# charlesknipp/sequential_monte_carlo

Measured on AMD Instinct MI355X. Metric: particle-steps/sec, higher is better.
Workload: dtype f64; 1 GPU; LinearGaussian1D bootstrap filter Nx=2^20 T=1000 (BASELINE configs[1]); n_theta_per_gpu=1, n_x=1048576, T=1000, seg=2048, resident_kernel=False, resampler=multinomial

## Files before the change

sequential_monte_carlo_amd/csrc/smc_kernels.h:

```cpp
#pragma once
#include "smc_spec.h"
#include <cstddef>
#include <type_traits>

namespace smc {

constexpr int WAVE = 64;
__host__ __device__ constexpr int lds_pad(int i) { return i + ((i >> 5) << 1); }
__host__ __device__ constexpr int lds_probe_off(int s) { return s >= 32 ? lds_pad(s - 32) + 31 : s - 1; }
__host__ __device__ constexpr int lds_step_inc(int s) { return s >= 32 ? lds_pad(s) : s; }
__host__ __device__ constexpr int lds_unpad(int pp) { return pp - 2 * (pp / 34); }
__host__ __device__ constexpr int lds_padded_len(int n) { return n + (n >> 4) + 8; }

typedef __attribute__((address_space(3))) const char lds_byte;
typedef __attribute__((address_space(3))) const uint64_t lds_u64;
typedef __attribute__((address_space(3))) const double lds_f64;
__device__ __forceinline__ lds_byte* lds_ptr(const void* p) { return (lds_byte*)p; }
__device__ __forceinline__ uint64_t lds_load_u64(lds_byte* p) { return *(lds_u64*)p; }

typedef unsigned long long nt_v2u64 __attribute__((ext_vector_type(2)));
template <class T>
__device__ __forceinline__ void store_out(T* p, const T& val) {
    static_assert(sizeof(T) == 16, "16-byte stores");
    __builtin_nontemporal_store(*reinterpret_cast<const nt_v2u64*>(&val), reinterpret_cast<nt_v2u64*>(p));
// ... 34 lines not shown
    int want_s2;
    const unsigned char* skip;
    const int32_t* order;
    const int32_t* n_active;
    int sum_np, sum_comp, sum_mom, sum_unw;
    uint64_t sum_p64[8];
    double* sum_q;
    double* sum_m;
    int abl;
    int prop_kind;
    unsigned long long* dbg;
    PropRow* prop;
};

#ifdef SMC_ABLATE
#define SMC_ABL(v, bit) (((v).abl >> (bit)) & 1)
#define SMC_STAMP(v, k)                                                                                   \
    do {                                                                                                  \
        if ((v).dbg && threadIdx.x == 0)                                                                  \
            (v).dbg[((size_t)blockIdx.y * gridDim.x + blockIdx.x) * 8 + (k)] = __builtin_amdgcn_s_memrealtime(); \
    } while (0)
#define SMC_CLOCK() __builtin_amdgcn_s_memrealtime()
#define SMC_STAMP_AT(v, k, clk)                                                                           \
    do {                                                                                                  \
        if ((v).dbg && threadIdx.x == 0)                                                                  \
            (v).dbg[((size_t)blockIdx.y * gridDim.x + blockIdx.x) * 8 + (k)] = (clk);                     \
    } while (0)
#define SMC_STAMP_START(v, t_draw, t_entry)                                                               \
    do {                                                                                                  \
        if ((v).dbg && threadIdx.x == 0) {                                                                \
            unsigned long long* d_ = (v).dbg + ((size_t)gridDim.y * gridDim.x + (size_t)blockIdx.y * gridDim.x + blockIdx.x) * 8; \
            d_[0] = (t_draw); d_[1] = (t_entry);                                                          \
        }                                                                                                 \
    } while (0)
#define SMC_ORDER_AFTER(x) asm volatile("" : : "v"(x))
#else
#define SMC_ORDER_AFTER(x) do { } while (0)
#define SMC_ABL(v, bit) 0
#define SMC_STAMP(v, k) do { } while (0)
#define SMC_STAMP_AT(v, k, clk) do { (void)(clk); } while (0)
#define SMC_CLOCK() 0ull
#define SMC_STAMP_START(v, t_draw, t_entry) do { (void)(t_draw); (void)(t_entry); } while (0)
#endif
__device__ __forceinline__ void host_emit(const FilterView& v, int th, double z, double logmu, double ess) {
    if (!v.host_out) return;
    v.host_out[th] = z;
    v.host_out[(size_t)v.ntheta + th] = logmu;
    v.host_out[2 * (size_t)v.ntheta + th] = ess;
    if (v.host_seq) {
        __threadfence_system();
        __hip_atomic_store(&v.host_out[3 * (size_t)v.ntheta + th], (double)v.host_seq, __ATOMIC_RELEASE, __HIP_MEMORY_SCOPE_SYSTEM);
    }
}
constexpr int QMAX = 8;
__host__ __device__ inline uint64_t order_key(double x) {
    const uint64_t b = d2bits(x);
    return (b >> 63) ? ~b : (b | 0x8000000000000000ULL);
}
__host__ __device__ inline double key_value(uint64_t k) { return bits2d((k >> 63) ? (k & 0x7fffffffffffffffULL) : ~k); }
__host__ __device__ inline uint64_t prob_to_u64(double p) {
    if (!(p > 0.0)) return 0;
    if (p >= 1.0) return ~(uint64_t)0;
    return (uint64_t)(p * TWO_P64);
}
struct Q7Rank { int64_t j; double g; };
__host__ __device__ inline Q7Rank q7_rank(int64_t n, double p) {
    const double h = (double)n * p + (1.0 - p);
    int64_t j = (int64_t)h;
    j = j > n - 1 ? n - 1 : (j < 1 ? 1 : j);
    double g = h - (double)j;
    g = g > 1.0 ? 1.0 : (g < 0.0 ? 0.0 : g);
    Q7Rank r; r.j = j; r.g = g;
    return r;
}
__host__ __device__ inline double q7_interp(double a, double b, double g) {
    const bool fin = (a - a == 0.0) && (b - b == 0.0);
    return fin ? a + g * (b - a) : (1.0 - g) * a + g * b;
}
__host__ __device__ inline double q7_level(double p) { return p > 0.0 ? (p < 1.0 ? p : 1.0) : 0.0; }


#define SMC_PRIO(ph) __builtin_amdgcn_s_setprio((short)(3 - (ph)))

template <int CTRL, int ROW_MASK>
__device__ __forceinline__ uint32_t dpp_u32(uint32_t old, uint32_t v) {
    return (uint32_t)__builtin_amdgcn_update_dpp((int)old, (int)v, CTRL, ROW_MASK, 0xf, false);
}
template <int CTRL>
__device__ __forceinline__ uint64_t dpp_add_u64(uint64_t v) {
    uint32_t lo = (uint32_t)v, hi = (uint32_t)(v >> 32);
#define SMC_DPP_ADD64(MOD)                                                                                  \
    asm volatile("s_nop 1\n\tv_add_co_u32_dpp %0, vcc, %0, %0 " MOD "\n\ts_nop 1\n\tv_addc_co_u32_dpp %1, vcc, %1, %1, vcc " MOD \
                 : "+v"(lo), "+v"(hi) : : "vcc")
    static_assert(CTRL == 0x111 || CTRL == 0x112 || CTRL == 0x114 || CTRL == 0x118 || CTRL == 0x142 || CTRL == 0x143, "DPP control");
    if (CTRL == 0x111) SMC_DPP_ADD64("row_shr:1 row_mask:0xf bank_mask:0xf bound_ctrl:1");
    if (CTRL == 0x112) SMC_DPP_ADD64("row_shr:2 row_mask:0xf bank_mask:0xf bound_ctrl:1");
    if (CTRL == 0x114) SMC_DPP_ADD64("row_shr:4 row_mask:0xf bank_mask:0xf bound_ctrl:1");
    if (CTRL == 0x118) SMC_DPP_ADD64("row_shr:8 row_mask:0xf bank_mask:0xf bound_ctrl:1");
    if (CTRL == 0x142) SMC_DPP_ADD64("row_bcast:15 row_mask:0xa bank_mask:0xf");
    if (CTRL == 0x143) SMC_DPP_ADD64("row_bcast:31 row_mask:0xc bank_mask:0xf");
#undef SMC_DPP_ADD64
    return ((uint64_t)hi << 32) | lo;
}
__device__ __forceinline__ uint64_t wave_incl_scan(uint64_t v, int ) {
    v = dpp_add_u64<0x111>(v);
    v = dpp_add_u64<0x112>(v);
    v = dpp_add_u64<0x114>(v);
    v = dpp_add_u64<0x118>(v);
    v = dpp_add_u64<0x142>(v);
    v = dpp_add_u64<0x143>(v);
    return v;
}
__device__ __forceinline__ uint32_t wave_incl_scan_u32(uint32_t v) {
    v += dpp_u32<0x111, 0xf>(0u, v);
    v += dpp_u32<0x112, 0xf>(0u, v);
    v += dpp_u32<0x114, 0xf>(0u, v);
    v += dpp_u32<0x118, 0xf>(0u, v);
    v += dpp_u32<0x142, 0xa>(0u, v);
    v += dpp_u32<0x143, 0xc>(0u, v);
    return v;
}
__device__ __forceinline__ uint64_t wave_incl_scan_52(uint64_t v) {
    const uint32_t lo = wave_incl_scan_u32((uint32_t)v & 0x3ffffffu);
    const uint32_t hi = wave_incl_scan_u32((uint32_t)(v >> 26));
    return ((uint64_t)hi << 26) + lo;
}
__device__ __forceinline__ uint64_t readlane_u64(uint64_t v, int l) {
    const uint32_t lo = (uint32_t)__builtin_amdgcn_readlane((int)(uint32_t)v, l);
    const uint32_t hi = (uint32_t)__builtin_amdgcn_readlane((int)(uint32_t)(v >> 32), l);
    return ((uint64_t)hi << 32) | lo;
}
__device__ __forceinline__ uint64_t wave_sum(uint64_t v) { return readlane_u64(wave_incl_scan(v, 0), WAVE - 1); }
template <int NW>
__device__ __forceinline__ void wave_totals(const uint64_t* tot, int lane, int wave, uint64_t& off, uint64_t& all) {
    static_assert(NW >= 1 && NW <= 16 && (NW & (NW - 1)) == 0, "wave count");
    uint64_t t = tot[lane & (NW - 1)];
    if (NW > 1) t = dpp_add_u64<0x111>(t);
    if (NW > 2) t = dpp_add_u64<0x112>(t);
    if (NW > 4) t = dpp_add_u64<0x114>(t);
    if (NW > 8) t = dpp_add_u64<0x118>(t);
    const int ws = __builtin_amdgcn_readfirstlane(wave);
    all = readlane_u64(t, NW - 1);
    const uint64_t prev = readlane_u64(t, ws > 0 ? ws - 1 : 0);
    off = ws > 0 ? prev : 0;
}

struct U128 {
    uint64_t lo, hi;
};
__device__ __forceinline__ U128 add128(U128 a, U128 b) {
    U128 r;
    r.lo = a.lo + b.lo;
    r.hi = a.hi + b.hi + (r.lo < a.lo ? 1u : 0u);
    return r;
}
__device__ __forceinline__ U128 sq128(uint64_t q) {
    U128 r;
    r.hi = __umul64hi(q, q);
    r.lo = q * q;
    return r;
}
template <int CTRL>
__device__ __forceinline__ U128 dpp_add_u128(U128 v) {
    uint32_t w0 = (uint32_t)v.lo, w1 = (uint32_t)(v.lo >> 32), w2 = (uint32_t)v.hi, w3 = (uint32_t)(v.hi >> 32);
#define SMC_DPP_ADD128(MOD)                                                                                       \
    asm volatile("s_nop 1\n\tv_add_co_u32_dpp %0, vcc, %0, %0 " MOD "\n\ts_nop 1\n\tv_addc_co_u32_dpp %1, vcc, %1, %1, vcc " MOD \
// ... 555 lines not shown
    double y;
    if constexpr (BYV) { prm = *prm0; y = yval; }
    else { prm = v.params[th]; y = v.y ? v.y[t] : yval; }
    PropRow prw;
    if constexpr (GUIDED) prw = v.prop[th];
    const uint32_t n32 = ea.n32;
    double xr[D] = {};
    if constexpr (COND) {
        uint32_t lane0 = 0u;
        if constexpr (D == 1) asm volatile("" : "+v"(lane0));
#pragma unroll
        for (int c = 0; c < D; ++c) xr[c] = xrow[(size_t)c * v.ntheta + th + lane0];
    }
    const uint64_t* Cprev = ea.C + (size_t)th * ((size_t)nseg * SEG);
    const double* xprev = v.x[cur];
    uint64_t* scr;
    SMC_PRIO(0);

    uint64_t F0 = 0, F1 = 0;
    if (MULTI && !SYS) {
        const uint64_t* Fb = ea.brow + (size_t)th * ((size_t)nseg + 1) + sb;
        F0 = Fb[0];
        F1 = Fb[1];
    }
    const TablePre tpre = (MULTI && !GTAB) ? table_preload<THREADS, RPT>(v, (const double*)ea.rec0, (const uint64_t*)ea.rec1, nseg, cur, th, emit_prev == 1 && sb == 0)
                                           : TablePre{-inf(), 0, 0, 0, -inf(), 0};
    unsigned long long t_draw = 0;
#pragma unroll
    for (int k = 0; k < NP; ++k) {
        if (SYS) { rr[2 * k] = rr[2 * k + 1] = 0; continue; }
        const uint32_t pg = (uint32_t)((seg0 >> 1) + tid + k * THREADS);
        rw[k] = draw(seed, pg, stream, t, SLOT_RESAMPLE);
        if (k == 0) {
            SMC_ORDER_AFTER(rw[0].v[3]);
            t_draw = SMC_CLOCK();
        }
        if (SMC_ABL(v, 3)) rw[k] = u32x4{{pg * 2654435761u, pg ^ t, pg * 40503u, ~pg}};
        rr[2 * k] = ((uint64_t)rw[k].v[1] << 32) | rw[k].v[0];
        rr[2 * k + 1] = ((uint64_t)rw[k].v[3] << 32) | rw[k].v[2];
    }
#ifdef SMC_ABLATE
    if (SMC_ABL(v, 8) && (blockIdx.x & 8)) {
        __builtin_amdgcn_s_sleep(127);
        __builtin_amdgcn_s_sleep(127);
    }
#endif
    const uint32_t m_blk = (seg0 + SEG < n32 ? seg0 + SEG : n32) - seg0;
    const bool ragged = seg0 + SEG > n32;
    uint32_t kk[NQ];
#pragma unroll
    for (int i = 0; i < NQ; ++i) kk[i] = 2 * (tid + (i >> 1) * THREADS) + (i & 1);
    if (ragged) {
        asm volatile("; ragged");
#pragma unroll
        for (int i = 0; i < NQ; ++i) kk[i] = (seg0 + kk[i] < n32 ? seg0 + kk[i] : n32 - 1) - seg0;
    }
    uint64_t Tg[NQ];

    constexpr bool SPEC = MULTI && NSTAGE == 3;
    ulonglong2 stg[NSTAGE][NP];
    int spec_lo = 0;
    if (SPEC) {
        spec_lo = sb - 1 < 0 ? 0 : sb - 1;
        spec_lo = spec_lo + NSTAGE > nseg ? (nseg - NSTAGE < 0 ? 0 : nseg - NSTAGE) : spec_lo;
#pragma unroll
        for (int sg = 0; sg < NSTAGE; ++sg) {
#pragma unroll
            for (int k = 0; k < NP; ++k) stg[sg][k] = ulonglong2{0, 0};
            if (spec_lo + sg < nseg) {
                const ulonglong2* src = reinterpret_cast<const ulonglong2*>(Cprev + (size_t)(spec_lo + sg) * SEG);
#pragma unroll
                for (int k = 0; k < NP; ++k) stg[sg][k] = src[tid + k * THREADS];
            }
        }
    }

    ulonglong2 stg1[NP];
    constexpr bool EARLY1 = D == 1;
#pragma unroll
    for (int k = 0; k < NP; ++k)
        stg1[k] = (!MULTI && EARLY1) ? reinterpret_cast<const ulonglong2*>(Cprev)[tid + k * THREADS] : ulonglong2{0, 0};

    constexpr bool LATE_Z = D >= 3 && NP >= 2 && !SYS;
    double z[NP][NZ][2];
#pragma unroll
    for (int k = 0; k < NP; ++k) {
        if (LATE_Z) break;
        const uint32_t pg = (uint32_t)((seg0 >> 1) + tid + k * THREADS);
#pragma unroll
        for (int c = 0; c < NZ; ++c) {
            if (SMC_ABL(v, 2)) { z[k][c][0] = 1e-3 * (double)(pg & 1023); z[k][c][1] = -z[k][c][0]; }
            else if (SMC_ABL(v, 6)) { const u32x4 w4 = draw(seed, pg, stream, t, SLOT_NORMAL0 + c); z[k][c][0] = 1e-9 * (double)w4.v[0]; z[k][c][1] = 1e-9 * (double)w4.v[2]; }
            else box_muller(draw(seed, pg, stream, t, SLOT_NORMAL0 + c), z[k][c][0], z[k][c][1]);
            if (SYS) asm volatile("" : "+v"(z[k][c][0]), "+v"(z[k][c][1]));
        }
    }


    uint64_t alive;
    uint64_t Sseg[NQ];
    int bseg[NQ];
    uint64_t* Cst = nullptr;
    int blo = 0;
    const int tab_p2 = GTAB ? 0 : v.nseg_p2;
    if (MULTI) {
        TableLds L = carve(smem, tab_p2);
        if (GTAB) {
            const size_t p2 = (size_t)1 << (32 - __builtin_clz((unsigned)(nseg - 1)));
            L.Dcum = (uint64_t*)ea.rec0 + (size_t)th * p2;
            L.sh = (int*)ea.rec1 + (size_t)th * p2;
        }
        scr = L.scr;
        uint64_t* sysw = L.scr + scr_words(THREADS, NP) - 8;
        if (SYS && tid == 0) {
            const u32x4 uw = draw(seed, 0u, stream, t, SLOT_SYS);
            sysw[0] = ((uint64_t)uw.v[1] << 32) | uw.v[0];
        }
        const bool emitter = emit_prev && sb == 0;
        const bool emit_totals = emitter && emit_prev == 2;
        const int s_hi = spec_lo + NSTAGE - 1 < v.nseg - 1 ? spec_lo + NSTAGE - 1 : v.nseg - 1;
        const bool use_fast = SPEC && (GTAB || ((!emitter || emit_totals) && v.nseg_p2 <= RPT * THREADS));
        uint64_t P0 = 0, Dc[NSTAGE];
        int shw[NSTAGE];
        if (GTAB) {
            alive = L.Dcum[v.nseg - 1];
            if (SPEC) {
                P0 = spec_lo ? L.Dcum[spec_lo - 1] : 0;
#pragma unroll
                for (int i = 0; i < NSTAGE; ++i) { Dc[i] = L.Dcum[spec_lo + i]; shw[i] = L.sh[spec_lo + i]; }
            }
            if (SYS) __syncthreads();
        } else if (use_fast) {
            double Kw;
            alive = window_prologue<THREADS, NSTAGE, RPT>(v, L.scr, tpre, spec_lo, P0, Dc, shw, Kw);
            if (emit_totals && tid == 0) emit_from_totals(v, th, Kw, alive, t == 1u, t - 1u);
        } else {
            alive = table_prologue<THREADS>(v, cur, th, L, emitter, t == 1u, t - 1u, RPT == 1 ? &tpre : nullptr);
        }
        SMC_STAMP(v, 1);
        SMC_PRIO(1);
        SysBase sbase{};
        uint64_t Tfirst, Tlast, lo_ = 0;
        if (SYS) {
            sbase = sys_base(alive, n32, v.inv_n, sysw[0], (uint64_t)seg0);
            Tfirst = sys_target(sbase, 0u);
            Tlast = sys_target(sbase, m_blk - 1);
        } else {
            mul64wide(F0, alive, Tfirst, lo_);
            mul64wide(F1, alive, Tlast, lo_);
        }
        bool fast = false;
        if (use_fast) {
            fast = (spec_lo == 0 || P0 <= Tfirst) && Tlast < Dc[s_hi - spec_lo];
            if (!fast && !GTAB) alive = table_prologue<THREADS>(v, cur, th, L, false, false, 0u, RPT == 1 ? &tpre : nullptr);
        }
        int b_lo = 0, b_hi = 0;
        if (fast || (SPEC && !use_fast && (spec_lo == 0 || L.Dcum[spec_lo - 1] <= Tfirst) && Tlast < L.Dcum[s_hi])) {
            b_lo = spec_lo;
            b_hi = s_hi;
        } else {
            for (int s = v.nseg_p2 >> 1; s >= 1; s >>= 1) {
                b_lo += (L.Dcum[b_lo + s - 1] <= Tfirst) ? s : 0;
                b_hi += (L.Dcum[b_hi + s - 1] <= Tlast) ? s : 0;
            }
            b_lo = b_lo < v.nseg ? b_lo : v.nseg - 1;
            b_hi = b_hi < v.nseg ? b_hi : v.nseg - 1;
            b_hi = b_hi < b_lo ? b_lo : b_hi;
        }
        int w0 = 1;
        while (w0 < b_hi - b_lo + 1) w0 <<= 1;
        Cst = (uint64_t*)(smem + (size_t)tab_p2 * 16 + scr_words(THREADS, NP) * 8);
        const bool spec_ok = SPEC && b_lo >= spec_lo && b_hi < spec_lo + NSTAGE;
        int st_lo = spec_lo;
        if (!spec_ok) {
            st_lo = b_lo;
// ... 28 lines not shown
                int r = 0;
                uint64_t base = P0;
                int shc = shw[0];
#pragma unroll
                for (int k = 0; k + 1 < NSTAGE; ++k) {
                    const bool up = Dc[k] <= Tg[i];
                    r += up ? 1 : 0;
                    base = up ? Dc[k] : base;
                    shc = up ? shw[k + 1] : shc;
                }
                bseg[i] = spec_lo + r;
                Sseg[i] = 0;
                Tg[i] = ((Tg[i] - base + 1) << shc) - 1;
            }
        } else {
            for (int s = w0 >> 1; s >= 1; s >>= 1) {
#pragma unroll
                for (int i = 0; i < NQ; ++i) {
                    const int c = pos[i] + s;
                    pos[i] = (c <= b_hi && L.Dcum[c - 1] <= Tg[i]) ? c : pos[i];
                }
            }
#pragma unroll
            for (int i = 0; i < NQ; ++i) {
                bseg[i] = pos[i];
                Sseg[i] = 0;
                const uint64_t base = bseg[i] ? L.Dcum[bseg[i] - 1] : 0;
                Tg[i] = sys_threshold(Tg[i] - base, L.sh[bseg[i]]);
            }
        }
    } else {
        const TableLds L = carve(smem, v.nseg_p2);
        scr = L.scr;
        if (emit_prev && sb == 0) table_prologue<THREADS>(v, cur, th, L, true, t == 1u, t - 1u);
        alive = ((const uint64_t*)ea.rec1)[(size_t)th * nseg];
#pragma unroll
        for (int i = 0; i < NQ; ++i) { bseg[i] = 0; Sseg[i] = alive; }
        if (SYS) {
            const int sh = seg_shift(0.0, 0.0, v.SH);
            const uint64_t Dtot = seg_Q(alive, sh);
            const u32x4 uw = draw(seed, 0u, stream, t, SLOT_SYS);
            const SysBase sbase = sys_base(Dtot, n32, v.inv_n, ((uint64_t)uw.v[1] << 32) | uw.v[0], 0u);
#pragma unroll
            for (int i = 0; i < NQ; ++i) Tg[i] = sys_threshold(sys_target(sbase, kk[i]), sh);
            alive = Dtot;
        }
    }

    SMC_STAMP(v, 2);
    SMC_STAMP_AT(v, 0, t_entry);
    SMC_STAMP_START(v, t_draw, t_entry);
    SMC_STAMP(v, 3);
    uint64_t T2[NQ];
#pragma unroll
    for (int i = 0; i < NQ; ++i) {
        uint64_t lo;
        if (SYS || MULTI) T2[i] = Tg[i];
        else mul64wide(rr[i], Sseg[i], T2[i], lo);
    }
    if (MULTI) {
#pragma unroll
        for (int sg = 0; sg < NSTAGE; ++sg)
#pragma unroll
            for (int k = 0; k < NP; ++k)
                *reinterpret_cast<ulonglong2*>(Cst + sg * SEGP + lds_pad(2 * (tid + k * THREADS))) = stg[sg][k];
        __syncthreads();
    } else {
        Cst = (uint64_t*)(smem + (size_t)v.nseg_p2 * 16 + scr_words(THREADS, NP) * 8);
#pragma unroll
        for (int k = 0; k < NP; ++k) {
            const ulonglong2 c2 = EARLY1 ? stg1[k] : reinterpret_cast<const ulonglong2*>(Cprev)[tid + k * THREADS];
            *reinterpret_cast<ulonglong2*>(Cst + lds_pad(2 * (tid + k * THREADS))) = c2;
        }
        __syncthreads();
    }
    SMC_STAMP(v, 4);
    SMC_PRIO(2);
    int pos[NQ];
#pragma unroll
    for (int i = 0; i < NQ; ++i) pos[i] = 0;
    if (SMC_ABL(v, 0)) {
#pragma unroll
        for (int i = 0; i < NQ; ++i) pos[i] = (int)(T2[i] & (SEG - 1));
    } else if (MULTI) {
        bool far = false;
        lds_byte* pb[NQ];
        lds_byte* pb0[NQ];
#pragma unroll
        for (int i = 0; i < NQ; ++i) {
            const int r = bseg[i] - blo;
            far |= r >= NSTAGE;
            pb0[i] = lds_ptr(Cst + (r < NSTAGE ? r : 0) * SEGP);
            pb[i] = pb0[i];
        }
#pragma unroll
        for (int s = SEG >> 1; s >= 1; s >>= 1) {
            uint64_t val[NQ];
#pragma unroll
            for (int i = 0; i < NQ; ++i) val[i] = lds_load_u64(pb[i] + 8 * lds_probe_off(s));
#pragma unroll
            for (int i = 0; i < NQ; ++i) pb[i] += (val[i] <= T2[i]) ? 8 * lds_step_inc(s) : 0;
        }
#pragma unroll
        for (int i = 0; i < NQ; ++i) pos[i] = lds_unpad((int)(pb[i] - pb0[i]) >> 3);
        if (__builtin_amdgcn_ballot_w64(far)) {
#pragma unroll
            for (int i = 0; i < NQ; ++i) {
                if (bseg[i] - blo >= NSTAGE) {
                    const uint64_t* Cb = Cprev + (size_t)bseg[i] * SEG;
                    int pp = 0;
                    for (int s = SEG >> 1; s >= 1; s >>= 1) pp += (Cb[pp + s - 1] <= T2[i]) ? s : 0;
                    pos[i] = pp;
                }
            }
        }
    } else {
        lds_byte* pb[NQ];
#pragma unroll
        for (int i = 0; i < NQ; ++i) pb[i] = lds_ptr(Cst);
#pragma unroll
        for (int s = SEG >> 1; s >= 1; s >>= 1) {
            uint64_t val[NQ];
#pragma unroll
            for (int i = 0; i < NQ; ++i) val[i] = lds_load_u64(pb[i] + 8 * lds_probe_off(s));
#pragma unroll
            for (int i = 0; i < NQ; ++i) pb[i] += (val[i] <= T2[i]) ? 8 * lds_step_inc(s) : 0;
        }
#pragma unroll
        for (int i = 0; i < NQ; ++i) pos[i] = lds_unpad((int)(pb[i] - lds_ptr(Cst)) >> 3);
    }
    SMC_STAMP(v, 5);
    uint32_t anc[NQ];
    double xp[NQ][D];
#pragma unroll
    for (int i = 0; i < NQ; ++i) {
        const uint32_t own = seg0 + 2 * (tid + (i >> 1) * THREADS) + (i & 1);
        uint32_t a = (uint32_t)bseg[i] * (uint32_t)SEG + (uint32_t)pos[i];
        if (!alive || ragged) {
            asm volatile("; collapsed or ragged");
            a = alive ? a : own;
            a = a < n32 ? a : n32 - 1;
        }
        anc[i] = a;
#pragma unroll
        for (int c = 0; c < D; ++c) xp[i][c] = SMC_ABL(v, 1) ? 0.25 * (double)(a & 7) : xprev[((size_t)c * v.ntheta + th) * v.npad + a];
    }

    uint32_t kst = 0;
    if constexpr (COND) kst = cond_slot(seed, stream, t, n32);

    double lw[NP][2];
#pragma unroll
    for (int k = 0; k < NP; ++k) {
        const uint32_t i0 = seg0 + 2 * (tid + k * THREADS);
        double xn[2][D];
        if (LATE_Z) {
            const uint32_t pg = (uint32_t)((seg0 >> 1) + tid + k * THREADS);
#pragma unroll
            for (int c = 0; c < NZ; ++c) box_muller(draw(seed, pg, stream, t, SLOT_NORMAL0 + c), z[k][c][0], z[k][c][1]);
        }
#pragma unroll
        for (int j = 0; j < 2; ++j) {
            double zz[NZ];
#pragma unroll
            for (int c = 0; c < NZ; ++c) zz[c] = z[k][c][j];
            if constexpr (MISS) {
                model_missing_step<MODEL>(prm, false, xp[2 * k + j], zz, xn[j]);
                lw[k][j] = 0.0;
            } else if constexpr (model_marginal<MODEL>::value) {
                lw[k][j] = model_marginal_step<MODEL>(prm, false, xp[2 * k + j], zz, y, xn[j]);
            } else if constexpr (GUIDED) {
                lw[k][j] = model_guided<MODEL>(prm, prw, xp[2 * k + j], zz, y, xn[j]);
            } else {
                model_transition<MODEL>(prm, xp[2 * k + j], zz, xn[j]);
                lw[k][j] = model_logobs<MODEL>(prm, xn[j], y);
            }
        }
        if constexpr (COND) {
            if (__builtin_amdgcn_ballot_w64((kst & ~1u) == i0)) {
                asm volatile("; retained slot");
                const double lwr = model_logobs<MODEL>(prm, xr, y);
                const uint32_t kprev = v.anc ? cond_slot(seed, stream, t - 1u, n32) : 0u;
#pragma unroll
                for (int j = 0; j < 2; ++j) {
                    const bool keep = (i0 + j) == kst;
#pragma unroll
                    for (int c = 0; c < D; ++c) xn[j][c] = keep ? xr[c] : xn[j][c];
                    lw[k][j] = keep ? lwr : lw[k][j];
                    anc[2 * k + j] = keep ? kprev : anc[2 * k + j];
                }
            }
        }
        if (ragged) {
            asm volatile("; ragged");
#pragma unroll
            for (int j = 0; j < 2; ++j)
                if (i0 + j >= n32) {
                    lw[k][j] = nan_mask();
#pragma unroll
                    for (int c = 0; c < D; ++c) xn[j][c] = 0.0;
                }
        }
#pragma unroll
        for (int c = 0; c < D; ++c) {
            double2 o;
            o.x = xn[0][c];
            o.y = xn[1][c];
            store_out(reinterpret_cast<double2*>(v.x[nxt] + ((size_t)c * v.ntheta + th) * v.npad + i0), o);
        }
        if (v.anc) {
            int2 o;
            o.x = (int)anc[2 * k];
// ... 170 lines not shown
```

sequential_monte_carlo_amd/csrc/smc_spec.h:

```cpp
#pragma once
#include <hip/hip_runtime.h>
#include <stdint.h>

#define SMC_HD __host__ __device__ __forceinline__

namespace smc {

constexpr int MODEL_LG1D = 1;
constexpr int MODEL_SV1D = 2;
constexpr int MODEL_UCSV3D = 3;
constexpr int MODEL_UCSV_RB = 4;
constexpr int NPARAM = 8;

constexpr int FIX_BITS = 48;
constexpr int MAX_SEG = 8192;
constexpr uint32_t SIM_STREAM = 0xFFFFFFFFu;
constexpr uint32_t SLOT_RESAMPLE = 0u;
constexpr uint32_t SLOT_NORMAL0 = 1u;
constexpr uint32_t SLOT_OBS = 8u;
constexpr uint32_t SLOT_COUNT = 9u;
constexpr uint32_t SLOT_SYS = 10u;
constexpr uint32_t SLOT_BREAK = 16u;
constexpr uint32_t SLOT_PMMH_Z = 32u;
constexpr uint32_t SLOT_PMMH_U = 33u;
// ... 104 lines not shown
    double y = __builtin_amdgcn_rcp(d);
    double e = fma(-d, y, 1.0);
    y = fma(y, e, y);
    e = fma(-d, y, 1.0);
    y = fma(y, e, y);
    const double q = n * y;
    const double r = fma(-d, q, n);
    return fma(r, y, q);
}
__device__ __forceinline__ double sqrt_moderate_or_negzero(double x) {
    const double y = __builtin_amdgcn_rsq(x);
    double g = x * y;
    double h = y * 0.5;
    const double r = fma(-h, g, 0.5);
    g = fma(g, r, g);
    double d = fma(-g, g, x);
    h = fma(h, r, h);
    g = fma(d, h, g);
    d = fma(-g, g, x);
    g = fma(d, h, g);
    return __builtin_fmax(g, -0.0);
}
#else
inline double div_moderate(double n, double d) { return n / d; }
inline double sqrt_moderate_or_negzero(double x) { return sqrt(x); }
#endif

SMC_HD double sp_exp_k(double x) { return rne(x * INV_LN2); }
SMC_HD double sp_exp_p(double x, double k);
SMC_HD double sp_exp_parts(double x, double& kout) {
    const double k = sp_exp_k(x);
    kout = k;
    return sp_exp_p(x, k);
}
SMC_HD double sp_exp_p(double x, double k) {
    double r = fma(-k, LN2_HI, x);
    r = fma(-k, LN2_LO, r);
    double p = 0x1.6124613a86d09p-33;
    p = SMC_FMAK(p, r, 0x1.1eed8eff8d898p-29);
    p = SMC_FMAK(p, r, 0x1.ae64567f544e4p-26);
    p = SMC_FMAK(p, r, 0x1.27e4fb7789f5cp-22);
    p = SMC_FMAK(p, r, 0x1.71de3a556c734p-19);
    p = SMC_FMAK(p, r, 0x1.a01a01a01a01ap-16);
    p = SMC_FMAK(p, r, 0x1.a01a01a01a01ap-13);
    p = SMC_FMAK(p, r, 0x1.6c16c16c16c17p-10);
    p = SMC_FMAK(p, r, 0x1.1111111111111p-7);
    p = SMC_FMAK(p, r, 0x1.5555555555555p-5);
    p = SMC_FMAK(p, r, 0x1.5555555555555p-3);
    p = SMC_FMAK(p, r, 0.5);
    p = SMC_FMAK(p, r, 1.0);
    p = SMC_FMAK(p, r, 1.0);
    return p;
}

SMC_HD double sp_exp(double x) {
#if defined(__HIP_DEVICE_COMPILE__)
    double k;
    const double p = sp_exp_parts(x, k);
    double r = scale2(p, (int)k);
    r = x > 709.0 ? inf() : r;
    r = x <= -708.0 ? 0.0 : r;
    return r;
#else
    if (x != x) return x;
    if (!(x > -708.0)) return 0.0;
    if (x > 709.0) return inf();
    double k;
    const double p = sp_exp_parts(x, k);
    return scale2(p, (int)k);
#endif
}

SMC_HD bool lw_alive(double l) { return l == l && (l < 0.0 ? -l : l) <= 7e8; }

SMC_HD uint64_t fix_weight(double p, double dk, int bits) {
    if (dk < -(double)(bits + 2)) return 0;
    return (uint64_t)rne_pos(p * pow2i(bits + (int)dk));
}
SMC_HD uint64_t fix_weight_i(double p, int dk, int bits) {
    if (dk < -(bits + 2)) return 0;
    return d2bits(p * pow2i(bits + dk) + 0x1p52) & 0x000fffffffffffffULL;
}

SMC_HD double sp_log_normal(double x, int e0) {
    const uint64_t b = d2bits(x);
    const uint64_t mant = b & 0x000fffffffffffffULL;
    const bool up = mant > (0x3ff6a09e667f3bcdULL & 0x000fffffffffffffULL);
    const int e = e0 + (int)((b >> 52) & 0x7ff) - 1023 + (up ? 1 : 0);
    const double m = bits2d(mant | (up ? 0x3fe0000000000000ULL : 0x3ff0000000000000ULL));
    const double f = m - 1.0;
    const double s = div_moderate(f, 2.0 + f);
    const double z = s * s;
    double R = 0x1.642c8590b2164p-4;
    R = SMC_FMAK(R, z, 0x1.8618618618618p-4);
    R = SMC_FMAK(R, z, 0x1.af286bca1af28p-4);
    R = SMC_FMAK(R, z, 0x1.e1e1e1e1e1e1ep-4);
    R = SMC_FMAK(R, z, 0x1.1111111111111p-3);
    R = SMC_FMAK(R, z, 0x1.3b13b13b13b14p-3);
    R = SMC_FMAK(R, z, 0x1.745d1745d1746p-3);
    R = SMC_FMAK(R, z, 0x1.c71c71c71c71cp-3);
    R = SMC_FMAK(R, z, 0x1.2492492492492p-2);
    R = SMC_FMAK(R, z, 0x1.999999999999ap-2);
    R = SMC_FMAK(R, z, 0x1.5555555555555p-1);
    R = R * z;
    const double dk = (double)e;
    return dk * LN2_HI - ((s * (f - R) - dk * LN2_LO) - f);
}

SMC_HD double sp_log(double x) {
    if (x != x || x < 0.0) return bits2d(0x7ff8000000000000ULL);
    if (x == 0.0) return -inf();
    if (x == inf()) return x;
    int e = 0;
    if (x < 0x1p-1022) { x *= 0x1p54; e = -54; }
    return sp_log_normal(x, e);
}

SMC_HD void sp_sincos2pi(double u, double& c, double& s) {
    const double a = 8.0 * u;
    const int oct = (int)a;
    const double g = fabs((double)(oct + (oct & 1)) - a);
    const double y = g * PIO4;
    const double z = y * y;
    double ps = 0x1.952c77030ad4ap-49;
    ps = SMC_FMAK(ps, z, -0x1.ae7f3e733b81fp-41);
    ps = SMC_FMAK(ps, z, 0x1.6124613a86d09p-33);
    ps = SMC_FMAK(ps, z, -0x1.ae64567f544e4p-26);
    ps = SMC_FMAK(ps, z, 0x1.71de3a556c734p-19);
    ps = SMC_FMAK(ps, z, -0x1.a01a01a01a01ap-13);
    ps = SMC_FMAK(ps, z, 0x1.1111111111111p-7);
    ps = SMC_FMAK(ps, z, -0x1.5555555555555p-3);
    const double sy = fma(y * z, ps, y);
    double pc = -0x1.6827863b97d97p-53;
    pc = SMC_FMAK(pc, z, 0x1.ae7f3e733b81fp-45);
    pc = SMC_FMAK(pc, z, -0x1.93974a8c07c9dp-37);
    pc = SMC_FMAK(pc, z, 0x1.1eed8eff8d898p-29);
    pc = SMC_FMAK(pc, z, -0x1.27e4fb7789f5cp-22);
    pc = SMC_FMAK(pc, z, 0x1.a01a01a01a01ap-16);
    pc = SMC_FMAK(pc, z, -0x1.6c16c16c16c17p-10);
    pc = SMC_FMAK(pc, z, 0x1.5555555555555p-5);
    pc = SMC_FMAK(pc, z, -0.5);
    const double cy = SMC_FMAK(z, pc, 1.0);
    const bool swap = ((oct + 1) & 2) != 0;
    double cc = swap ? sy : cy;
    double ss = swap ? cy : sy;
    const uint64_t cb = d2bits(cc), sb = d2bits(ss);
    const uint32_t ch = xor_and((uint32_t)(cb >> 32), ((uint32_t)oct << 29) + 0x40000000u, 0x80000000u);
    const uint32_t sh = xor_and((uint32_t)(sb >> 32), (uint32_t)oct << 29, 0x80000000u);
    c = bits2d(((uint64_t)ch << 32) | (uint32_t)cb);
    s = bits2d(((uint64_t)sh << 32) | (uint32_t)sb);
}

SMC_HD void box_muller(const u32x4& w, double& z0, double& z1) {
    const double u1 = fma((double)w.v[1], 0x1p-32, (double)((w.v[0] >> 11) + 1u) * TWO_M53);
    const double u2 = fma((double)w.v[3], 0x1p-32, (double)(w.v[2] >> 11) * TWO_M53);
    const double r = sqrt_moderate_or_negzero(-2.0 * sp_log_normal(u1, 0));
    double c, s;
    sp_sincos2pi(u2, c, s);
    z0 = r * c;
    z1 = r * s;
}

SMC_HD void mul64wide(uint64_t a, uint64_t b, uint64_t& hi, uint64_t& lo) {
#if defined(__HIP_DEVICE_COMPILE__)
    hi = __umul64hi(a, b);
    lo = a * b;
#else
    const unsigned __int128 p = (unsigned __int128)a * b;
    hi = (uint64_t)(p >> 64);
    lo = (uint64_t)p;
#endif
}

SMC_HD double uniform53(const u32x4& w) {
    return (double)(((((uint64_t)w.v[1] << 32) | w.v[0]) >> 11) + 1) * TWO_M53;
}
SMC_HD uint64_t gamma_fix(uint64_t seed, uint32_t w, uint32_t stream, uint32_t t, int64_t m) {
    const double d = (double)m - 1.0 / 3.0, c = 1.0 / sqrt(9.0 * d);
    double G = d;
    for (uint32_t it = 0; it < 8; ++it) {
        double x, z1;
        box_muller(draw(seed, w, stream, t, SLOT_BREAK + 2 * it), x, z1);
        const double vv = 1.0 + c * x;
        if (!(vv > 0.0)) continue;
        const double v3 = vv * vv * vv, x2 = x * x;
        const double u = uniform53(draw(seed, w, stream, t, SLOT_BREAK + 2 * it + 1));
        if (u < 1.0 - 0.0331 * (x2 * x2) || sp_log(u) < 0.5 * x2 + d * ((1.0 - v3) + sp_log(v3))) {
            G = d * v3;
            break;
        }
    }
    const uint64_t g = (uint64_t)rne_pos(G * 0x1p32);
    return g ? g : 1;
}
SMC_HD uint64_t exp1_fix(uint64_t seed, uint32_t w, uint32_t stream, uint32_t t) {
    const uint64_t e = (uint64_t)rne_pos(-sp_log(uniform53(draw(seed, w, stream, t, SLOT_BREAK + 1))) * 0x1p32);
    return e ? e : 1;
}
SMC_HD uint64_t div_frac64(uint64_t P, uint64_t S) {
    uint64_t rem = P, q = 0;
    for (int i = 0; i < 64; ++i) {
        rem <<= 1;
        q <<= 1;
        if (rem >= S) { rem -= S; q |= 1; }
    }
    return q;
}

SMC_HD void divmod_u64_u32(uint64_t D, uint32_t N, double inv, uint64_t& q, uint32_t& r) {
    if ((N & (N - 1u)) == 0u) {
        const int sft = __builtin_ctz(N);
        q = D >> sft;
        r = (uint32_t)(D & (uint64_t)(N - 1u));
        return;
    }
    uint64_t q1 = (uint64_t)((double)D * inv);
    int64_t r1 = (int64_t)(D - q1 * (uint64_t)N);
    const int64_t q2 = (int64_t)floor((double)r1 * inv);
    q1 += (uint64_t)q2;
    r1 -= q2 * (int64_t)N;
    if (r1 < 0) { q1 -= 1; r1 += N; }
    if (r1 >= (int64_t)N) { q1 += 1; r1 -= N; }
    q = q1;
    r = (uint32_t)r1;
}
struct SysBase {
    uint64_t Tbase, dq;
    double inv;
    uint32_t ra, dr, n;
};
SMC_HD SysBase sys_base(uint64_t Dtot, uint32_t n, double inv, uint64_t u, uint64_t j0) {
    uint64_t v0, lo;
    mul64wide(u, Dtot, v0, lo);
    SysBase sb;
    sb.n = n;
    sb.inv = inv;
    uint64_t q0, qa;
    uint32_t r0;
    divmod_u64_u32(Dtot, n, sb.inv, sb.dq, sb.dr);
    divmod_u64_u32(v0, n, sb.inv, q0, r0);
    divmod_u64_u32((uint64_t)r0 + j0 * (uint64_t)sb.dr, n, sb.inv, qa, sb.ra);
    sb.Tbase = q0 + j0 * sb.dq + qa;
    return sb;
// ... 687 lines not shown
```

Measured before the change: 94.95 billion particle-steps/s.

## Interleave last Box-Muller normals with LDS binary-search levels in D==1 path

Splits the Box-Muller transform into ten slices held in an explicit state struct, and spreads the slices for the last particle group across the levels of the LDS binary search. Scheduling barriers pin each slice between a level's LDS probe load and its compare. The aim is to hide LDS load latency behind independent FP64 arithmetic. The cost is higher register pressure from the live BmState and a more rigid instruction schedule.

```diff
diff --git a/sequential_monte_carlo_amd/csrc/smc_kernels.h b/sequential_monte_carlo_amd/csrc/smc_kernels.h
--- a/sequential_monte_carlo_amd/csrc/smc_kernels.h
+++ b/sequential_monte_carlo_amd/csrc/smc_kernels.h
@@ -140,6 +140,43 @@
 
 #define SMC_PRIO(ph) __builtin_amdgcn_s_setprio((short)(3 - (ph)))
 
+#ifndef SMC_FILL_HEAD
+#define SMC_FILL_HEAD 0
+#endif
+static_assert(SMC_FILL_HEAD >= 0 && SMC_FILL_HEAD < BM_NSLICE, "slices kept at the head");
+__host__ __device__ constexpr int bm_first(int l, int nlev) { return SMC_FILL_HEAD + (l * (BM_NSLICE - SMC_FILL_HEAD) + nlev - 1) / nlev; }
+__host__ __device__ constexpr int search_levels(int seg) { return seg <= 1 ? 0 : 1 + search_levels(seg >> 1); }
+template <int I>
+__device__ __forceinline__ void bm_pin(BmState& b) {
+    if constexpr (I < 0) asm volatile("" : "+v"(b.w.v[0]), "+v"(b.w.v[1]), "+v"(b.w.v[2]), "+v"(b.w.v[3]));
+    else if constexpr (I == 0) asm volatile("" : "+v"(b.u1), "+v"(b.u2));
+    else if constexpr (I == 1) asm volatile("" : "+v"(b.u2), "+v"(b.e), "+v"(b.f), "+v"(b.s));
+    else if constexpr (I == 2) asm volatile("" : "+v"(b.u2), "+v"(b.e), "+v"(b.f), "+v"(b.s), "+v"(b.zl), "+v"(b.R));
+    else if constexpr (I == 3 || I == 4) asm volatile("" : "+v"(b.u2), "+v"(b.x));
+    else if constexpr (I == 5) asm volatile("" : "+v"(b.x), "+v"(b.oct), "+v"(b.y), "+v"(b.zs), "+v"(b.ps));
+    else if constexpr (I == 6 || I == 7) asm volatile("" : "+v"(b.x), "+v"(b.oct), "+v"(b.zs), "+v"(b.sy), "+v"(b.pc));
+    else if constexpr (I == 8) asm volatile("" : "+v"(b.x), "+v"(b.z0), "+v"(b.z1));
+    else asm volatile("" : "+v"(b.z0), "+v"(b.z1));
+}
+template <int NLEV, int NZ, int L = 0>
+__device__ __forceinline__ void bm_level(int l, BmState (&b)[NZ]) {
+    if constexpr (L < NLEV) {
+        if (l == L) {
+            constexpr int A = bm_first(L, NLEV), B = bm_first(L + 1, NLEV);
+            if constexpr (A < B) {
+#pragma unroll
+                for (int c = 0; c < NZ; ++c) {
+                    bm_pin<A - 1>(b[c]);
+                    bm_slices<A, B>(b[c]);
+                    bm_pin<B - 1>(b[c]);
+                }
+            }
+        } else {
+            bm_level<NLEV, NZ, L + 1>(l, b);
+        }
+    }
+}
+
 template <int CTRL, int ROW_MASK>
 __device__ __forceinline__ uint32_t dpp_u32(uint32_t old, uint32_t v) {
     return (uint32_t)__builtin_amdgcn_update_dpp((int)old, (int)v, CTRL, ROW_MASK, 0xf, false);
@@ -861,7 +898,13 @@
         stg1[k] = (!MULTI && EARLY1) ? reinterpret_cast<const ulonglong2*>(Cprev)[tid + k * THREADS] : ulonglong2{0, 0};
 
     constexpr bool LATE_Z = D >= 3 && NP >= 2 && !SYS;
+    constexpr bool FILL = D == 1 && !SYS;
+    static_assert(!(FILL && LATE_Z), "late normals are not interleaved");
+    constexpr int NLEV = search_levels(SEG);
+    static_assert(!FILL || (NLEV >= 1 && bm_first(0, NLEV) == SMC_FILL_HEAD && bm_first(NLEV, NLEV) == BM_NSLICE), "slice map of the search");
+    const bool fill = FILL && !SMC_ABL(v, 2) && !SMC_ABL(v, 6);
     double z[NP][NZ][2];
+    BmState bm[NZ];
 #pragma unroll
     for (int k = 0; k < NP; ++k) {
         if (LATE_Z) break;
@@ -870,6 +913,11 @@
         for (int c = 0; c < NZ; ++c) {
             if (SMC_ABL(v, 2)) { z[k][c][0] = 1e-3 * (double)(pg & 1023); z[k][c][1] = -z[k][c][0]; }
             else if (SMC_ABL(v, 6)) { const u32x4 w4 = draw(seed, pg, stream, t, SLOT_NORMAL0 + c); z[k][c][0] = 1e-9 * (double)w4.v[0]; z[k][c][1] = 1e-9 * (double)w4.v[2]; }
+            else if (FILL && k == NP - 1) {
+                bm[c].w = draw(seed, pg, stream, t, SLOT_NORMAL0 + c);
+                bm_slices<0, SMC_FILL_HEAD>(bm[c]);
+                bm_pin<SMC_FILL_HEAD - 1>(bm[c]);
+            }
             else box_muller(draw(seed, pg, stream, t, SLOT_NORMAL0 + c), z[k][c][0], z[k][c][1]);
             if (SYS) asm volatile("" : "+v"(z[k][c][0]), "+v"(z[k][c][1]));
         }
@@ -1064,6 +1112,10 @@
     if (SMC_ABL(v, 0)) {
 #pragma unroll
         for (int i = 0; i < NQ; ++i) pos[i] = (int)(T2[i] & (SEG - 1));
+        if (fill) {
+#pragma unroll
+            for (int c = 0; c < NZ; ++c) bm_slices<SMC_FILL_HEAD, BM_NSLICE>(bm[c]);
+        }
     } else if (MULTI) {
         bool far = false;
         lds_byte* pb[NQ];
@@ -1076,10 +1128,15 @@
             pb[i] = pb0[i];
         }
 #pragma unroll
-        for (int s = SEG >> 1; s >= 1; s >>= 1) {
+        for (int s = SEG >> 1, l = 0; s >= 1; s >>= 1, ++l) {
             uint64_t val[NQ];
 #pragma unroll
             for (int i = 0; i < NQ; ++i) val[i] = lds_load_u64(pb[i] + 8 * lds_probe_off(s));
+            if constexpr (FILL) {
+                __builtin_amdgcn_sched_barrier(0);
+                if (fill) bm_level<NLEV>(l, bm);
+                __builtin_amdgcn_sched_barrier(0);
+            }
 #pragma unroll
             for (int i = 0; i < NQ; ++i) pb[i] += (val[i] <= T2[i]) ? 8 * lds_step_inc(s) : 0;
         }
@@ -1101,15 +1158,24 @@
 #pragma unroll
         for (int i = 0; i < NQ; ++i) pb[i] = lds_ptr(Cst);
 #pragma unroll
-        for (int s = SEG >> 1; s >= 1; s >>= 1) {
+        for (int s = SEG >> 1, l = 0; s >= 1; s >>= 1, ++l) {
             uint64_t val[NQ];
 #pragma unroll
             for (int i = 0; i < NQ; ++i) val[i] = lds_load_u64(pb[i] + 8 * lds_probe_off(s));
+            if constexpr (FILL) {
+                __builtin_amdgcn_sched_barrier(0);
+                if (fill) bm_level<NLEV>(l, bm);
+                __builtin_amdgcn_sched_barrier(0);
+            }
 #pragma unroll
             for (int i = 0; i < NQ; ++i) pb[i] += (val[i] <= T2[i]) ? 8 * lds_step_inc(s) : 0;
         }
 #pragma unroll
         for (int i = 0; i < NQ; ++i) pos[i] = lds_unpad((int)(pb[i] - lds_ptr(Cst)) >> 3);
+    }
+    if (fill) {
+#pragma unroll
+        for (int c = 0; c < NZ; ++c) { z[NP - 1][c][0] = bm[c].z0; z[NP - 1][c][1] = bm[c].z1; }
     }
     SMC_STAMP(v, 5);
     uint32_t anc[NQ];
diff --git a/sequential_monte_carlo_amd/csrc/smc_spec.h b/sequential_monte_carlo_amd/csrc/smc_spec.h
--- a/sequential_monte_carlo_amd/csrc/smc_spec.h
+++ b/sequential_monte_carlo_amd/csrc/smc_spec.h
@@ -210,29 +210,38 @@
     return d2bits(p * pow2i(bits + dk) + 0x1p52) & 0x000fffffffffffffULL;
 }
 
-SMC_HD double sp_log_normal(double x, int e0) {
+SMC_HD void log_split(double x, int e0, int& e, double& f) {
     const uint64_t b = d2bits(x);
     const uint64_t mant = b & 0x000fffffffffffffULL;
     const bool up = mant > (0x3ff6a09e667f3bcdULL & 0x000fffffffffffffULL);
-    const int e = e0 + (int)((b >> 52) & 0x7ff) - 1023 + (up ? 1 : 0);
+    e = e0 + (int)((b >> 52) & 0x7ff) - 1023 + (up ? 1 : 0);
     const double m = bits2d(mant | (up ? 0x3fe0000000000000ULL : 0x3ff0000000000000ULL));
-    const double f = m - 1.0;
+    f = m - 1.0;
+}
+constexpr double LOG_R0 = 0x1.642c8590b2164p-4;
+constexpr int LOG_NC = 10;
+constexpr double LOG_C[LOG_NC] = {0x1.8618618618618p-4, 0x1.af286bca1af28p-4, 0x1.e1e1e1e1e1e1ep-4, 0x1.1111111111111p-3,
+                                  0x1.3b13b13b13b14p-3, 0x1.745d1745d1746p-3, 0x1.c71c71c71c71cp-3, 0x1.2492492492492p-2,
+                                  0x1.999999999999ap-2, 0x1.5555555555555p-1};
+#define SMC_POLY_STEPS(name, C)                                        \
+    template <int A, int B>                                            \
+    SMC_HD double name(double p, double z) {                           \
+        if constexpr (A < B) return name<A + 1, B>(SMC_FMAK(p, z, C[A]), z); \
+        else return p;                                                 \
+    }
+SMC_POLY_STEPS(log_poly, LOG_C)
+SMC_HD double log_combine(int e, double f, double s, double Rz) {
+    const double dk = (double)e;
+    return dk * LN2_HI - ((s * (f - Rz) - dk * LN2_LO) - f);
+}
+SMC_HD double sp_log_normal(double x, int e0) {
+    int e;
+    double f;
+    log_split(x, e0, e, f);
     const double s = div_moderate(f, 2.0 + f);
     const double z = s * s;
-    double R = 0x1.642c8590b2164p-4;
-    R = SMC_FMAK(R, z, 0x1.8618618618618p-4);
-    R = SMC_FMAK(R, z, 0x1.af286bca1af28p-4);
-    R = SMC_FMAK(R, z, 0x1.e1e1e1e1e1e1ep-4);
-    R = SMC_FMAK(R, z, 0x1.1111111111111p-3);
-    R = SMC_FMAK(R, z, 0x1.3b13b13b13b14p-3);
-    R = SMC_FMAK(R, z, 0x1.745d1745d1746p-3);
-    R = SMC_FMAK(R, z, 0x1.c71c71c71c71cp-3);
-    R = SMC_FMAK(R, z, 0x1.2492492492492p-2);
-    R = SMC_FMAK(R, z, 0x1.999999999999ap-2);
-    R = SMC_FMAK(R, z, 0x1.5555555555555p-1);
-    R = R * z;
-    const double dk = (double)e;
-    return dk * LN2_HI - ((s * (f - R) - dk * LN2_LO) - f);
+    const double R = log_poly<0, LOG_NC>(LOG_R0, z);
+    return log_combine(e, f, s, R * z);
 }
 
 SMC_HD double sp_log(double x) {
@@ -244,31 +253,27 @@
     return sp_log_normal(x, e);
 }
 
-SMC_HD void sp_sincos2pi(double u, double& c, double& s) {
+SMC_HD void sc_reduce(double u, int& oct, double& y, double& z) {
     const double a = 8.0 * u;
-    const int oct = (int)a;
+    oct = (int)a;
     const double g = fabs((double)(oct + (oct & 1)) - a);
-    const double y = g * PIO4;
-    const double z = y * y;
-    double ps = 0x1.952c77030ad4ap-49;
-    ps = SMC_FMAK(ps, z, -0x1.ae7f3e733b81fp-41);
-    ps = SMC_FMAK(ps, z, 0x1.6124613a86d09p-33);
-    ps = SMC_FMAK(ps, z, -0x1.ae64567f544e4p-26);
-    ps = SMC_FMAK(ps, z, 0x1.71de3a556c734p-19);
-    ps = SMC_FMAK(ps, z, -0x1.a01a01a01a01ap-13);
-    ps = SMC_FMAK(ps, z, 0x1.1111111111111p-7);
-    ps = SMC_FMAK(ps, z, -0x1.5555555555555p-3);
-    const double sy = fma(y * z, ps, y);
-    double pc = -0x1.6827863b97d97p-53;
-    pc = SMC_FMAK(pc, z, 0x1.ae7f3e733b81fp-45);
-    pc = SMC_FMAK(pc, z, -0x1.93974a8c07c9dp-37);
-    pc = SMC_FMAK(pc, z, 0x1.1eed8eff8d898p-29);
-    pc = SMC_FMAK(pc, z, -0x1.27e4fb7789f5cp-22);
-    pc = SMC_FMAK(pc, z, 0x1.a01a01a01a01ap-16);
-    pc = SMC_FMAK(pc, z, -0x1.6c16c16c16c17p-10);
-    pc = SMC_FMAK(pc, z, 0x1.5555555555555p-5);
-    pc = SMC_FMAK(pc, z, -0.5);
-    const double cy = SMC_FMAK(z, pc, 1.0);
+    y = g * PIO4;
+    z = y * y;
+}
+constexpr double SIN_P0 = 0x1.952c77030ad4ap-49;
+constexpr int SIN_NC = 7;
+constexpr double SIN_C[SIN_NC] = {-0x1.ae7f3e733b81fp-41, 0x1.6124613a86d09p-33, -0x1.ae64567f544e4p-26, 0x1.71de3a556c734p-19,
+                                  -0x1.a01a01a01a01ap-13, 0x1.1111111111111p-7, -0x1.5555555555555p-3};
+constexpr double COS_P0 = -0x1.6827863b97d97p-53;
+constexpr int COS_NC = 8;
+constexpr double COS_C[COS_NC] = {0x1.ae7f3e733b81fp-45, -0x1.93974a8c07c9dp-37, 0x1.1eed8eff8d898p-29, -0x1.27e4fb7789f5cp-22,
+                                  0x1.a01a01a01a01ap-16, -0x1.6c16c16c16c17p-10, 0x1.5555555555555p-5, -0.5};
+SMC_POLY_STEPS(sin_poly, SIN_C)
+SMC_POLY_STEPS(cos_poly, COS_C)
+#undef SMC_POLY_STEPS
+SMC_HD double sc_sin(double y, double z, double ps) { return fma(y * z, ps, y); }
+SMC_HD double sc_cos(double z, double pc) { return SMC_FMAK(z, pc, 1.0); }
+SMC_HD void sc_place(int oct, double sy, double cy, double& c, double& s) {
     const bool swap = ((oct + 1) & 2) != 0;
     double cc = swap ? sy : cy;
     double ss = swap ? cy : sy;
@@ -278,15 +283,72 @@
     c = bits2d(((uint64_t)ch << 32) | (uint32_t)cb);
     s = bits2d(((uint64_t)sh << 32) | (uint32_t)sb);
 }
-
+SMC_HD void sp_sincos2pi(double u, double& c, double& s) {
+    int oct;
+    double y, z;
+    sc_reduce(u, oct, y, z);
+    const double sy = sc_sin(y, z, sin_poly<0, SIN_NC>(SIN_P0, z));
+    const double cy = sc_cos(z, cos_poly<0, COS_NC>(COS_P0, z));
+    sc_place(oct, sy, cy, c, s);
+}
+
+struct BmState {
+    u32x4 w;
+    double u1, u2;
+    int e;
+    double f, s, zl, R;
+    double x;
+    int oct;
+    double y, zs, ps, pc, sy;
+    double z0, z1;
+};
+constexpr int BM_NSLICE = 10;
+template <int I>
+SMC_HD void bm_slice(BmState& b) {
+    static_assert(I >= 0 && I < BM_NSLICE, "slice index");
+    if constexpr (I == 0) {
+        b.u1 = fma((double)b.w.v[1], 0x1p-32, (double)((b.w.v[0] >> 11) + 1u) * TWO_M53);
+        b.u2 = fma((double)b.w.v[3], 0x1p-32, (double)(b.w.v[2] >> 11) * TWO_M53);
+    } else if constexpr (I == 1) {
+        log_split(b.u1, 0, b.e, b.f);
+        b.s = div_moderate(b.f, 2.0 + b.f);
+    } else if constexpr (I == 2) {
+        b.zl = b.s * b.s;
+        b.R = log_poly<0, 7>(LOG_R0, b.zl);
+    } else if constexpr (I == 3) {
+        b.R = log_poly<7, LOG_NC>(b.R, b.zl);
+        b.x = -2.0 * log_combine(b.e, b.f, b.s, b.R * b.zl);
+    } else if constexpr (I == 4) {
+        b.x = sqrt_moderate_or_negzero(b.x);
+    } else if constexpr (I == 5) {
+        sc_reduce(b.u2, b.oct, b.y, b.zs);
+        b.ps = sin_poly<0, 4>(SIN_P0, b.zs);
+    } else if constexpr (I == 6) {
+        b.ps = sin_poly<4, SIN_NC>(b.ps, b.zs);
+        b.sy = sc_sin(b.y, b.zs, b.ps);
+        b.pc = cos_poly<0, 2>(COS_P0, b.zs);
+    } else if constexpr (I == 7) {
+        b.pc = cos_poly<2, COS_NC>(b.pc, b.zs);
+    } else if constexpr (I == 8) {
+        sc_place(b.oct, b.sy, sc_cos(b.zs, b.pc), b.z0, b.z1);
+    } else {
+        b.z0 = b.x * b.z0;
+        b.z1 = b.x * b.z1;
+    }
+}
+template <int A, int B>
+SMC_HD void bm_slices(BmState& b) {
+    if constexpr (A < B) {
+        bm_slice<A>(b);
+        bm_slices<A + 1, B>(b);
+    }
+}
 SMC_HD void box_muller(const u32x4& w, double& z0, double& z1) {
-    const double u1 = fma((double)w.v[1], 0x1p-32, (double)((w.v[0] >> 11) + 1u) * TWO_M53);
-    const double u2 = fma((double)w.v[3], 0x1p-32, (double)(w.v[2] >> 11) * TWO_M53);
-    const double r = sqrt_moderate_or_negzero(-2.0 * sp_log_normal(u1, 0));
-    double c, s;
-    sp_sincos2pi(u2, c, s);
-    z0 = r * c;
-    z1 = r * s;
+    BmState b;
+    b.w = w;
+    bm_slices<0, BM_NSLICE>(b);
+    z0 = b.z0;
+    z1 = b.z1;
 }
 
 SMC_HD void mul64wide(uint64_t a, uint64_t b, uint64_t& hi, uint64_t& lo) {
```

Measured after the change: 97.03 billion particle-steps/s (median of 6 runs). +2.2%, better.
